# AkiRusProd/numpy-nn-model

Hardware: AMD Instinct MI355X
Metric: samples/sec training step (higher is better)
Workload: dtype f32; 1 GPU; C4: GPT-tiny d512 L6 H8 d_ff2048 vocab15000 training step, batch 64 x seq 256 per GPU, Adam(1.5e-4), dropout 0; global_batch=64, seq_len=256, parallelism=dp1, launch=hipGraph replay, scaling=weak: 64 sequences per GPU

## Files before the change

include/neunet_hip.h:

```cpp
#ifndef NEUNET_HIP_H
#define NEUNET_HIP_H

#include <stdint.h>

#ifdef __cplusplus
extern "C" {
#endif

typedef void* nnhipStream_t;

#define NNHIP_OK 0
#define NNHIP_EINVAL (-1)
#define NNHIP_EALIGN (-2)
#define NNHIP_ENOMEM (-3)
#define NNHIP_EDEVICE (-5)

int nnhipVersion(void);
const char* nnhipGetLastErrorString(void);
int nnhipCleanup(void);
int nnhipDeviceError(void);
int nnhipClearDeviceError(void);
int nnhipRaiseDeviceErrorForTest(int32_t code, nnhipStream_t stream);
int nnhipWorkspaceReserve(int64_t bytes);
int nnhipWorkspaceLock(int locked);

int nnhipSetGemmMode(int mode);
int nnhipGetGemmMode(void);
int nnhipSetGemmLockstep(int enable);
int nnhipGetGemmLockstep(void);
int64_t nnhipGemmLaunchCount(int family);

int nnhipLinearModuleForward(const float* X, const float* W, const float* b, float* O,
                             int64_t rows, int64_t in_features, int64_t out_features,
                             nnhipStream_t stream);
int nnhipLinearModuleBackward(const float* X, const float* W, const float* dO, float* dX,
                              float* dW, float* db, int64_t rows, int64_t in_features,
                              int64_t out_features, nnhipStream_t stream);
int nnhipLinearModuleForwardEx(const float* X, const float* W, const float* b, const float* addend, float* O,
                               int64_t rows, int64_t in_features, int64_t out_features, nnhipStream_t stream);
int nnhipLinearModuleBackwardEx(const float* X, const float* W, const float* dO, const float* dX_addend, float* dX,
                                float* dW, float* db, int64_t rows, int64_t in_features, int64_t out_features,
                                nnhipStream_t stream);

#define NNHIP_LINEAR_GEMV_MAX_ROWS 8
int nnhipLinearGemvForward(const float* X, const float* W, const float* b, const float* addend, float* O, int64_t rows,
                           int64_t in_features, int64_t out_features, nnhipStream_t stream);
int nnhipSetLinearGemv(int enable);
int nnhipGetLinearGemv(void);

int nnhipWeightGradDefer(int32_t enable, nnhipStream_t stream);
int nnhipWeightGradFlush(nnhipStream_t stream);
int nnhipWeightGradFlushGemms(nnhipStream_t stream);
// ... 387 lines not shown
```

numpy-nn-model_amd/csrc/common.h:

```cpp
#pragma once
#include <hip/hip_runtime.h>
#include <stdint.h>
#include <stdio.h>

#include "../../include/neunet_hip.h"

namespace nnhip {

constexpr int kWave = 64;

void set_last_error(const char* fmt, ...);
int hip_status(hipError_t e, const char* what);

#define NNHIP_CHECK_ARG(cond, code, ...)      \
    do {                                       \
        if (!(cond)) {                         \
            nnhip::set_last_error(__VA_ARGS__); \
            return (code);                     \
        }                                      \
    } while (0)

#define NNHIP_LAUNCH_CHECK(name)                          \
    do {                                                  \
        hipError_t _e = hipGetLastError();                \
// ... 2 lines not shown

inline bool aligned16(const void* p) { return (reinterpret_cast<uintptr_t>(p) & 15u) == 0; }
inline bool aligned8(const void* p) { return (reinterpret_cast<uintptr_t>(p) & 7u) == 0; }
inline bool aligned4(const void* p) { return (reinterpret_cast<uintptr_t>(p) & 3u) == 0; }
inline int64_t ceil_div(int64_t a, int64_t b) { return (a + b - 1) / b; }

void* workspace(size_t bytes);
void* workspace_arena(int which, size_t bytes);
bool workspace_locked();
bool wgrad_defer_on();
int conv_reduce_flush(void* stream);
void conv_reduce_cleanup();
int colsum_flush(void* stream);
void colsum_cleanup();
struct WgradJob {
    const float* A; const float* B; float* C; float* asum;
    int64_t M, N, K;
};

const float* zero_block();
constexpr int kSyncWords = 1024;
enum SyncSlot { SYNC_CE = 0, SYNC_MLP = 24 };
unsigned* sync_words();
enum DeviceErrorCode { NNHIP_DEVERR_NONE = 0, NNHIP_DEVERR_MLP_BARRIER = 1, NNHIP_DEVERR_LSTM_SHAPE = 2, NNHIP_DEVERR_KVCACHE_FULL = 3, NNHIP_DEVERR_RECURRENT_SHAPE = 4 };
unsigned* device_error_word();
int device_error_status(const char* who);
int serialize_shared_state(hipStream_t st);
void shared_state_done(hipStream_t st);
struct SharedStateUse {
    hipStream_t st;
    explicit SharedStateUse(hipStream_t s) : st(s) {}
    ~SharedStateUse() { shared_state_done(st); }
    SharedStateUse(const SharedStateUse&) = delete;
    SharedStateUse& operator=(const SharedStateUse&) = delete;
};

template <int CTRL>
__device__ __forceinline__ float dpp_f32(float v) {
    return __builtin_bit_cast(float, __builtin_amdgcn_update_dpp(0, __builtin_bit_cast(int, v), CTRL, 0xF, 0xF, false));
}
template <int CTRL>
__device__ __forceinline__ int dpp_i32(int v) { return __builtin_amdgcn_update_dpp(0, v, CTRL, 0xF, 0xF, false); }
constexpr int kDppXor1 = 0xB1, kDppXor2 = 0x4E, kDppHalfMirror = 0x141, kDppMirror = 0x140;
__device__ __forceinline__ float readlane_f32(float v, int lane) {
    return __builtin_bit_cast(float, __builtin_amdgcn_readlane(__builtin_bit_cast(int, v), lane));
}
// ... 97 lines not shown
```

numpy-nn-model_amd/csrc/gemm.hip:

```cpp
#include <stdlib.h>

#include <type_traits>

#include "gemm_common.h"

namespace nnhip {

__device__ int g_gemm_progress[8192];


template <int BK, bool AKC, bool BKC, bool VEC, bool SUM>
__device__ __forceinline__ void gemm_k_loop(f32x16 (&acc)[2][2], float4 (&ra)[BK / 8], float4 (&rb)[BK / 8], float4& cs,
                                            float* __restrict__ smem, const float* __restrict__ A,
                                            const float* __restrict__ B, const GemmParams& p, int nk, int64_t kbeg,
                                            int64_t kend, int64_t m0, int64_t n0, int tid, int wm, int wn, int l31,
                                            int lh, const float* __restrict__ Z) {
    using TA = Tile<BK, AKC>;
    using TB = Tile<BK, BKC>;
    constexpr int STAGE = TA::SIZE + TB::SIZE;
    constexpr int NLD = 2 * (BK / 8);
    constexpr int NMF = 16 * (BK / 8);
    int cur = 0;
    for (int kt = 0; kt < nk; ++kt) {
        const bool more = kt + 1 < nk;
// ... 107 lines not shown
                                         int l31, int lh) {
    using TA = Tile<BK, AKC>;
    using TB = Tile<BK, BKC>;
    const float* As = smem + cur * (TA::SIZE + TB::SIZE);
    const float* Bs = As + TA::SIZE;
#pragma unroll 1
    for (int g = g0; g < BK / 8; ++g) {
        float a[2][4], b[2][4];
#pragma unroll
        for (int i = 0; i < 2; ++i) {
            frag<BK, AKC>(a[i], As, wm * 64 + i * 32 + l31, g, lh);
            frag<BK, BKC>(b[i], Bs, wn * 64 + i * 32 + l31, g, lh);
        }
#pragma unroll
        for (int j = 0; j < 4; ++j)
#pragma unroll
            for (int i = 0; i < 2; ++i)
#pragma unroll
                for (int n = 0; n < 2; ++n)
                    acc[i][n] = __builtin_amdgcn_mfma_f32_32x32x2f32(a[i][j], b[n][j], acc[i][n], 0, 0, 0);
    }
}

template <int BK, bool AKC, bool BKC, bool VEC, bool CS = false>
__device__ __forceinline__ void gemm_f32_block(const GemmParams& p, const int L, const int by, float* __restrict__ smem) {
    static_assert(!CS || !AKC, "row sums of A are only implemented for an outer-major A");
    using TA = Tile<BK, AKC>;

    const int tid = threadIdx.x;
    const int lane = tid & 63, wave = tid >> 6;
    const int wm = wave >> 1, wn = wave & 1;
    const int l31 = lane & 31, lh = lane >> 5;
#ifdef GEMM_PROF
    long long ts_[5];
    ts_[0] = clock64();
#define GP_STAMP(i) ts_[i] = clock64()
#else
#define GP_STAMP(i) do {} while (0)
#endif
    const int tiles = p.tiles_m * p.tiles_n;
    const int split = L / tiles;
    const int t = L - split * tiles;
    constexpr int GM = 8;
    const int in_group = GM * p.tiles_n;
    const int grp = t / in_group;
    const int first_m = grp * GM;
    const int gsz = min(p.tiles_m - first_m, GM);
// ... 95 lines not shown
            gemm_k_step<BK, AKC, BKC, CS>(acc, ra2, rb2, ra, rb, cs, csf, smem, cur, rsa, rsb, ka_of(kt + 2), kb_of(kt + 2), offa, offb,
                                          tid, wm, wn, l31, lh);
            cur ^= 1;
        }
        if (plock) __builtin_amdgcn_s_setprio(0);
        if (has_tail) {
            tail_mma<BK, AKC, BKC>(acc, smem, cur, (BK - rem) >> 3, wm, wn, l31, lh);
            __syncthreads();
        }
        GP_STAMP(2);
    } else {
        const int nk = (int)((kend - kbeg + BK - 1) / BK);
        const float* __restrict__ Z = p.zeros;
        g2r<BK, AKC, VEC>(ra, A, p.lda, p.M, kend, m0, kbeg, tid, nk > 0, Z);
        g2r<BK, BKC, VEC>(rb, B, p.ldb, p.N, kend, n0, kbeg, tid, nk > 0, Z);
        r2s<BK, AKC>(ra, smem, tid);
        r2s<BK, BKC>(rb, smem + TA::SIZE, tid);
        __syncthreads();
        gemm_k_loop<BK, AKC, BKC, VEC, CS>(acc, ra, rb, cs, smem, A, B, p, nk, kbeg, kend, m0, n0, tid, wm, wn, l31, lh, Z);
    }

#ifdef GEMM_PROF
    long long ets_[5] = {0, 0, 0, 0, 0};
    gemm_epilogue<CS>(acc, p, smem, cs, tid, wave, lane, wm, wn, l31, lh, m0, n0, tn, split, c_off, ets_);
#else
    gemm_epilogue<CS>(acc, p, smem, cs, tid, wave, lane, wm, wn, l31, lh, m0, n0, tn, split, c_off);
#endif
#ifdef GEMM_PROF
    if constexpr (VEC) {
        GP_STAMP(3);
        __builtin_amdgcn_s_waitcnt(0);
        GP_STAMP(4);
        if (p.prof && lane == 0) {
            long long* o = p.prof + ((int64_t)blockIdx.x * 4 + wave) * 12;
            o[0] = ts_[0]; o[1] = ts_[1]; o[2] = ts_[2]; o[3] = ts_[3]; o[4] = ts_[4];
            for (int q_ = 0; q_ < 5; ++q_) o[5 + q_] = ets_[q_];
            o[10] = __builtin_amdgcn_s_getreg((31 << 11) | 4);
            o[11] = ((long long)__builtin_amdgcn_s_getreg((31 << 11) | 20) << 32) | (unsigned)(tm * 65536 + tn);
        }
    }
#endif
}

template <int BK, bool AKC, bool BKC, bool VEC, bool CS = false>
__global__ __launch_bounds__(NT, (BK <= 16) ? 3 : 2) void gemm_f32_kernel(const GemmParams p) {
    extern __shared__ __attribute__((aligned(16))) float smem[];
    gemm_f32_block<BK, AKC, BKC, VEC, CS>(p, xcd_order((int)blockIdx.x, (int)gridDim.x), (int)blockIdx.y, smem);
}

template <int BK>
__global__ __launch_bounds__(NT, 2) void gemm_f32_group_kernel(const GemmGroup g) {
    extern __shared__ __attribute__((aligned(16))) float smem[];
    const int b = (int)blockIdx.x;
    const int L = g.by_job ? b : xcd_order(b, (int)gridDim.x);
    int i = 0;
#pragma unroll
    for (int j = 1; j < GEMM_GROUP_MAX; ++j)
        if (j < g.n && L >= g.start[j]) i = j;
    const int local = L - g.start[i];
    gemm_f32_block<BK, false, false, true, true>(g.p[i], g.by_job ? xcd_order(local, g.start[i + 1] - g.start[i]) : local, 0, smem);
}

struct ReduceArgs {
    const float* slab; float* C; float* preact; const float* bias;
    int64_t M, N, ldc;
    int splitk, act; float beta, alpha;
    const float* asum_slab; float* asum; const float* addend; int asum_blocks, vec;
    const float* dswish; int dact;
};
__device__ __forceinline__ void splitk_reduce_body(const ReduceArgs& r, const int blk, const int nblk) {
    const float* __restrict__ slab = r.slab; float* __restrict__ C = r.C; float* __restrict__ preact = r.preact;
    const float* __restrict__ bias = r.bias; const float* __restrict__ asum_slab = r.asum_slab; float* __restrict__ asum = r.asum;
    const float* __restrict__ addend = r.addend; const float* __restrict__ dswish = r.dswish;
    const int64_t M = r.M, N = r.N, ldc = r.ldc;
    const int splitk = r.splitk, act = r.act, vec = r.vec, dact = r.dact;
    const float beta = r.beta, alpha = r.alpha;
    const int64_t total = M * N;
    const int main_blocks = nblk - r.asum_blocks;
    if (blk >= main_blocks) {
        const int64_t i = (int64_t)(blk - main_blocks) * blockDim.x + threadIdx.x;
        if (i < M) {
            float s = 0.f;
            for (int k = 0; k < splitk; ++k) s += asum_slab[(int64_t)k * M + i];
// ... 80 lines not shown
        hipError_t e = hipFuncSetAttribute(reinterpret_cast<const void*>(kern),
                                           hipFuncAttributeMaxDynamicSharedMemorySize, (int)lds);
        if (e != hipSuccess) return hip_status(e, "hipFuncSetAttribute(gemm)");
        attr_set = true;
    }
    dim3 grid((unsigned)(p.tiles_m * p.tiles_n * p.splitk), (unsigned)batch);
    hipLaunchKernelGGL(kern, grid, dim3(NT), lds, st, p);
    NNHIP_LAUNCH_CHECK("gemm_f32_kernel");
    return 0;
}

int gemm_f32_ex(const float* A, const float* B, float* C, const float* bias, float* preact, int64_t M,
                int64_t N, int64_t K, int64_t lda, int64_t ldb, int64_t ldc, bool a_kmajor, bool b_kmajor,
                int64_t batch1, int64_t sA, int64_t sB, int64_t sC, int64_t batch2, int64_t sA2,
                int64_t sB2, int64_t sC2, float alpha, int act, float beta, hipStream_t st, float* asum = nullptr,
                const float* addend = nullptr, const float* dswish = nullptr, int dact = 1);

int gemm_bf3_launch(const GemmParams& p, bool a_kmajor, bool b_kmajor, bool vec, bool cs, int64_t batch, hipStream_t st);
int gemm_bf3_group_launch(const GemmGroup& g, int blocks, hipStream_t st);
long long linear_gemv_launches();
static int gemm_f32_uneven_split(const float* A, const float* B, float* C, float* asum, int64_t M, int64_t N, int64_t K, int64_t lda,
                                 int64_t ldb, int64_t ldc, int64_t K1, hipStream_t st);
static long long g_gemm_launches[4] = {0, 0, 0, 0};
static int g_gemm_lockstep = []() { const char* e = getenv("NNHIP_GEMM_LOCKSTEP"); return e && atoi(e) == 1 ? 1 : 0; }();
static int g_gemm_mode = -1;
static int gemm_mode() {
    if (g_gemm_mode < 0) {
        const char* e = getenv("NNHIP_GEMM_MODE");
        g_gemm_mode = (e && (atoi(e) == 1 || e[0] == 'b')) ? 1 : 0;
    }
    return g_gemm_mode;
}

bool gemm_pst_wanted(int64_t M, int64_t N, int64_t K, int64_t lda, int64_t ldb, int64_t ldc, const float* A, const float* B,
                     const float* C, const float* bias, bool b_kmajor, int act, const float* preact, const float* dswish, int dact);
int gemm_pst(const float* A, const float* B, float* C, const float* bias, float* preact, int64_t M, int64_t N, int64_t K,
             int64_t lda, int64_t ldb, int64_t ldc, bool b_kmajor, float alpha, int act, float beta, const float* dswish, int dact,
             hipStream_t st);
int gemm_small_linear_backward(const float* X, const float* W, const float* dO, float* dX, float* dW, float* db, int64_t rows,
                               int64_t in, int64_t out, const float* addend, const float* dact_arg, int dact, float beta,
                               hipStream_t st);
bool gemm_small_wanted(int64_t M, int64_t N, int64_t K, int64_t batch, int64_t lda, int64_t ldb, bool a_kmajor, bool b_kmajor);
int gemm_small(const float* A, const float* B, float* C, const float* bias, float* preact, int64_t M, int64_t N, int64_t K,
               int64_t lda, int64_t ldb, int64_t ldc, bool a_kmajor, bool b_kmajor, float alpha, int act, float beta,
               float* asum, const float* addend, const float* dact_arg, int dact, hipStream_t st);

#ifdef GEMM_PROF
static long long* g_gemm_prof = nullptr;
// ... 196 lines not shown
    constexpr int BK = 32;
    const size_t floats = 2 * (size_t)(M * N + (asum ? M : 0));
    float* slab = static_cast<float*>(workspace(floats * sizeof(float)));
    if (!slab) { set_last_error("split-K workspace allocation failed"); return NNHIP_ENOMEM; }
    const float* zeros = zero_block();
    if (!zeros) { set_last_error("zero block allocation failed"); return NNHIP_ENOMEM; }
    float* asum_slab = asum ? slab + 2 * (size_t)(M * N) : nullptr;
    GemmGroup g{};
    g.n = 2;
    g.by_job = 1;
    const int tiles_m = (int)ceil_div(M, BM), tiles_n = (int)ceil_div(N, BN), tiles = tiles_m * tiles_n;
    for (int i = 0; i < 2; ++i) {
        GemmParams& p = g.p[i];
        const int64_t k0 = i ? K1 : 0, kn = i ? K - K1 : K1;
        p.A = A + k0 * lda; p.B = B + k0 * ldb; p.C = C; p.M = M; p.N = N; p.K = kn; p.lda = lda; p.ldb = ldb; p.ldc = ldc;
        p.batch2 = 1; p.alpha = 1.f; p.beta = 1.f; p.tiles_m = tiles_m; p.tiles_n = tiles_n;
        p.k_per_split = ceil_div(kn, BK) * BK;
        p.splitk = 2;
        p.slab = slab + (size_t)i * M * N; p.zeros = zeros; p.cvec = 1; p.asum = asum;
        p.asum_slab = asum ? asum_slab + (size_t)i * M : nullptr;
        g.start[i] = i * tiles;
    }
    for (int i = 2; i <= GEMM_GROUP_MAX; ++i) g.start[i] = 2 * tiles;
    if (int rc = launch_group(g, 2 * tiles, st)) return rc;
    const int rvec = (ldc & 3) == 0 && aligned16(C);
    const int64_t work = rvec ? M * N / 4 : M * N;
    const int blocks = (int)(ceil_div(work, 256) < 2048 ? ceil_div(work, 256) : 2048);
    const int asum_blocks = asum ? (int)ceil_div(M, 256) : 0;
    const ReduceArgs r{slab, C, nullptr, nullptr, M, N, ldc, 2, ACT_NONE, 1.f, 1.f, asum_slab, asum, nullptr, asum_blocks, rvec, nullptr, 0};
    hipLaunchKernelGGL(splitk_reduce_kernel, dim3(blocks + asum_blocks), dim3(256), 0, st, r);
    NNHIP_LAUNCH_CHECK("splitk_reduce_kernel");
    return 0;
}

static int64_t wgrad_chunk(int64_t K) {
    static const int64_t forced = []() { const char* e = getenv("NNHIP_WGRAD_CHUNK"); return (int64_t)(e ? atoi(e) : 0); }();
    if (forced > 0) return ceil_div(forced, (int64_t)32) * 32;
    const int64_t c = ceil_div(ceil_div(K, (int64_t)4), (int64_t)32) * 32;
    return c < 1024 ? 1024 : c;
}
bool gemm_f32_wgrad_group_ok(const WgradJob& j) {
    static const int on = []() { const char* e = getenv("NNHIP_WGRAD_GROUP_KERNEL"); return e ? atoi(e) : 1; }();
    if (!on) return false;
    if (j.M <= 0 || j.N <= 0 || j.K < 4096 || (j.K & 7)) return false;
    if ((j.M & 3) || (j.N & 3) || !aligned16(j.A) || !aligned16(j.B) || !aligned16(j.C)) return false;
    if (j.K * j.M + 128 >= ((int64_t)1 << 30) || j.K * j.N + 128 >= ((int64_t)1 << 30)) return false;
    const int64_t tiles = ceil_div(j.M, BM) * ceil_div(j.N, BN);
    return tiles <= 256;
}

int gemm_f32_wgrad_group(const WgradJob* jobs, int n, hipStream_t st) {
    if (n <= 0) return 0;
    if (n > GEMM_GROUP_MAX) {
        for (int i = 0; i < n; i += GEMM_GROUP_MAX)
            if (int rc = gemm_f32_wgrad_group(jobs + i, n - i < GEMM_GROUP_MAX ? n - i : GEMM_GROUP_MAX, st)) return rc;
        return 0;
    }
    GemmGroup g{};
    ReduceGroup rg{};
    size_t floats = 0;
    for (int i = 0; i < n; ++i) {
        const WgradJob& j = jobs[i];
        const int64_t kps = wgrad_chunk(j.K);
        floats += (size_t)ceil_div(j.K, kps) * (size_t)(j.M * j.N + (j.asum ? j.M : 0));
    }
    float* slab = static_cast<float*>(workspace_arena(1, floats * sizeof(float)));
    if (!slab) { set_last_error("grouped dW workspace allocation failed"); return NNHIP_ENOMEM; }
    const float* zeros = zero_block();
    if (!zeros) { set_last_error("zero block allocation failed"); return NNHIP_ENOMEM; }
    g.n = rg.n = n;
    int blocks = 0, rblocks = 0;
    for (int i = 0; i < n; ++i) {
        const WgradJob& j = jobs[i];
        GemmParams& p = g.p[i];
        p = GemmParams{};
        p.A = j.A; p.B = j.B; p.C = j.C; p.M = j.M; p.N = j.N; p.K = j.K; p.lda = j.M; p.ldb = j.N; p.ldc = j.N;
        p.batch2 = 1; p.alpha = 1.f; p.beta = 1.f;
        p.tiles_m = (int)ceil_div(j.M, BM); p.tiles_n = (int)ceil_div(j.N, BN);
        p.k_per_split = wgrad_chunk(j.K);
        p.splitk = (int)ceil_div(j.K, p.k_per_split);
        p.slab = slab; p.zeros = zeros; p.cvec = 1; p.asum = j.asum;
        slab += (size_t)p.splitk * j.M * j.N;
        if (j.asum) { p.asum_slab = slab; slab += (size_t)p.splitk * j.M; }
        g.start[i] = blocks;
        blocks += p.tiles_m * p.tiles_n * p.splitk;
        const int64_t work = j.M * j.N / 4;
        const int main_blocks = (int)(ceil_div(work, 256) < 2048 ? ceil_div(work, 256) : 2048);
        const int asum_blocks = j.asum ? (int)ceil_div(j.M, 256) : 0;
        rg.r[i] = ReduceArgs{p.slab, j.C, nullptr, nullptr, j.M, j.N, j.N, p.splitk, ACT_NONE, 1.f, 1.f, p.asum_slab, j.asum, nullptr,
                             asum_blocks, 1, nullptr, 0};
        rg.start[i] = rblocks;
        rblocks += main_blocks + asum_blocks;
    }
    for (int i = n; i <= GEMM_GROUP_MAX; ++i) { g.start[i] = blocks; rg.start[i] = rblocks; }
    g_gemm_launches[gemm_mode() == 1 ? 3 : 0] += n;
    if (int rc = launch_group(g, blocks, st)) return rc;
    hipLaunchKernelGGL(splitk_reduce_group_kernel, dim3((unsigned)rblocks), dim3(256), 0, st, rg);
    NNHIP_LAUNCH_CHECK("splitk_reduce_group_kernel");
    return 0;
}

}

extern "C" int nnhipSetGemmMode(int mode) {
    NNHIP_CHECK_ARG(mode == 0 || mode == 1, NNHIP_EINVAL, "nnhipSetGemmMode: 0 = exact fp32 MFMA, 1 = split-bf16 (bf16x3)");
    nnhip::g_gemm_mode = mode;
    return 0;
}
extern "C" int nnhipGetGemmMode(void) { return nnhip::gemm_mode(); }
extern "C" int nnhipSetGemmLockstep(int enable) {
    NNHIP_CHECK_ARG(enable == 0 || enable == 1, NNHIP_EINVAL, "nnhipSetGemmLockstep: 0 = off (default), 1 = the two blocks of a CU keep step");
    nnhip::g_gemm_lockstep = enable;
    return 0;
}
extern "C" int nnhipGetGemmLockstep(void) { return nnhip::g_gemm_lockstep; }
extern "C" int64_t nnhipGemmLaunchCount(int family) {
    if (family == 4) return (int64_t)nnhip::linear_gemv_launches();
    return family >= 0 && family < 4 ? (int64_t)nnhip::g_gemm_launches[family] : -1;
}

extern "C" int nnhipGemmF32Ex(const float* A, const float* B, float* C, const float* bias, int64_t M,
                              int64_t N, int64_t K, int64_t lda, int64_t ldb, int64_t ldc, int a_kmajor,
                              int b_kmajor, int64_t batch1, int64_t sA1, int64_t sB1, int64_t sC1,
                              int64_t batch2, int64_t sA2, int64_t sB2, int64_t sC2, float alpha,
                              nnhipStream_t stream) {
    NNHIP_CHECK_ARG(A && B && C, NNHIP_EINVAL, "nnhipGemmF32Ex: null operand");
    NNHIP_CHECK_ARG(M >= 0 && N >= 0 && K >= 0 && batch1 >= 0 && batch2 >= 1, NNHIP_EINVAL, "nnhipGemmF32Ex: bad size");
    NNHIP_CHECK_ARG(batch1 * batch2 <= 65535, NNHIP_EINVAL, "nnhipGemmF32Ex: batch1*batch2 must be <= 65535");
    NNHIP_CHECK_ARG(nnhip::aligned4(A) && nnhip::aligned4(B) && nnhip::aligned4(C), NNHIP_EALIGN,
                    "nnhipGemmF32Ex: pointers must be 4-byte aligned");
    return nnhip::gemm_f32_ex(A, B, C, bias, nullptr, M, N, K, lda, ldb, ldc, a_kmajor != 0, b_kmajor != 0,
                              batch1, sA1, sB1, sC1, batch2, sA2, sB2, sC2, alpha, nnhip::ACT_NONE, 1.f,
                              static_cast<hipStream_t>(stream));
}

extern "C" int nnhipGemmF32(const float* A, const float* B, float* C, const float* bias, int64_t M,
                            int64_t N, int64_t K, int64_t lda, int64_t ldb, int64_t ldc,
                            int a_kmajor, int b_kmajor, int64_t batch, int64_t strideA,
// ... 11 lines not shown
```

numpy-nn-model_amd/csrc/gemm_common.h:

```cpp
#pragma once
#include "common.h"

namespace nnhip {

typedef float f32x16 __attribute__((ext_vector_type(16)));

enum { ACT_NONE = 0, ACT_SWISH = 1, ACT_RELU = 2, ACT_SIGMOID = 3,
       ACT_SWISH_D = 4 };

struct GemmParams {
    const float* A;
    const float* B;
    float* C;
    const float* bias;
    float* preact;
    int64_t M, N, K, lda, ldb, ldc, sA, sB, sC;
    int64_t sA2, sB2, sC2;
    int batch2;
    float alpha;
    int tiles_m, tiles_n, splitk;
    int lockstep = 0;
#ifdef GEMM_PROF
    long long* prof;
#endif
    int64_t k_per_split;
    float* slab;
    const float* zeros;
    int cvec;
    int act;
    float beta;
    const float* dswish;
    int dact;
    const float* addend;
    float* asum;
    float* asum_slab;
};

constexpr int BM = 128, BN = 128, NT = 256;

template <int BK, bool KC, bool VEC>
__device__ __forceinline__ void g2r(float4 (&r)[BK / 8], const float* __restrict__ P, int64_t ld,
                                    int64_t R, int64_t Kend, int64_t r0, int64_t k0, int tid, bool live,
                                    const float* __restrict__ Z) {
#pragma unroll
    for (int p = 0; p < BK / 8; ++p) {
        const int idx = tid + NT * p;
        int64_t gr, gk;
        const float* src;
        if constexpr (KC) {
            const int rr = idx / (BK / 4), k4 = (idx % (BK / 4)) * 4;
            gr = r0 + rr; gk = k0 + k4;
            src = P + gr * ld + gk;
        } else {
            const int kk = idx / 32, r4 = (idx % 32) * 4;
            gk = k0 + kk; gr = r0 + r4;
            src = P + gk * ld + gr;
        }
        if constexpr (VEC) {
// ... 54 lines not shown
#pragma unroll
    for (int p = 0; p < BK / 8; ++p) {
        const int idx = tid + NT * p;
        if constexpr (KC) {
            const int rr = idx / (BK / 4), k4 = (idx % (BK / 4)) * 4;
            const int64_t rc = min((int64_t)rr, R - 1 - r0);
            off[p] = (unsigned)((rc * ld + k4) * 4);
        } else {
            const int kk = idx / 32, r4 = (idx % 32) * 4;
            const int64_t rc = min((int64_t)r4, R - 4 - r0);
            off[p] = (unsigned)(((int64_t)kk * ld + rc) * 4);
        }
    }
}
template <int BK>
__device__ __forceinline__ void g2r_fast(float4 (&r)[BK / 8], __amdgpu_buffer_rsrc_t rs, unsigned koff, const unsigned (&off)[BK / 8]) {
#pragma unroll
    for (int p = 0; p < BK / 8; ++p) {
        const u32x4_ t = __builtin_amdgcn_raw_buffer_load_b128(rs, off[p], koff, 0);
        r[p].x = __uint_as_float(t.x); r[p].y = __uint_as_float(t.y); r[p].z = __uint_as_float(t.z); r[p].w = __uint_as_float(t.w);
    }
}

template <bool CS>
__device__ __forceinline__ void gemm_epilogue(f32x16 (&acc)[2][2], const GemmParams& p, float* __restrict__ smem, float4 cs,
                                              int tid, int wave, int lane, int wm, int wn, int l31, int lh, int64_t m0,
                                              int64_t n0, int tn, int split, int64_t c_off, long long* ets = nullptr) {
    const bool to_slab = p.splitk > 1;
    if constexpr (CS) {
        if (p.asum && tn == 0) {
            *reinterpret_cast<float4*>(&smem[(tid >> 5) * 128 + (tid & 31) * 4]) = cs;
            __syncthreads();
            if (tid < 128) {
                float t = 0.f;
#pragma unroll
                for (int r = 0; r < 8; ++r) t += smem[r * 128 + tid];
                if (m0 + tid < p.M) (to_slab ? p.asum_slab + (int64_t)split * p.M : p.asum)[m0 + tid] = t;
            }
            __syncthreads();
        }
    }
    float* __restrict__ C = to_slab ? p.slab + (int64_t)split * p.M * p.N : p.C + c_off;
    const int64_t ldc = to_slab ? p.N : p.ldc;
    if (p.cvec) {
        constexpr int ELD = 68;
        float* E = smem + wave * (32 * ELD);
        const int er = lane >> 4, ec = (lane & 15) * 4;
        const int64_t col = n0 + wn * 64 + ec;
        const bool col_ok = col < p.N;
        float4 bv = make_float4(0.f, 0.f, 0.f, 0.f);
        if (!to_slab && p.bias && col_ok) bv = *reinterpret_cast<const float4*>(p.bias + col);
        const float* __restrict__ extra = to_slab ? nullptr : (p.addend ? p.addend : p.dswish);
        const bool is_add = p.addend != nullptr;
        float4 ex[8];
        auto fetch_extra = [&](int i, int it) {
            const int64_t row = m0 + wm * 64 + i * 32 + it * 4 + er;
            ex[it] = make_float4(0.f, 0.f, 0.f, 0.f);
            if (row < p.M && col_ok) ex[it] = *reinterpret_cast<const float4*>(extra + c_off + row * ldc + col);
        };
        if (extra) {
#pragma unroll
            for (int it = 0; it < 8; ++it) fetch_extra(0, it);
        }
#ifdef GEMM_PROF
        if (ets) ets[0] = clock64();
#endif
#pragma unroll
        for (int i = 0; i < 2; ++i) {
#pragma unroll
            for (int n = 0; n < 2; ++n)
#pragma unroll
                for (int e = 0; e < 16; ++e)
                    E[((e & 3) + 8 * (e >> 2) + 4 * lh) * ELD + n * 32 + l31] = acc[i][n][e];
            __builtin_amdgcn_s_waitcnt(0xc07f);
            __builtin_amdgcn_wave_barrier();
#ifdef GEMM_PROF
// ... 18 lines not shown
                                v.z = x.z > 0.f ? v.z : 0.f; v.w = x.w > 0.f ? v.w : 0.f;
                            } else if (p.dact == 3) {
                                v.x *= x.x; v.y *= x.y; v.z *= x.z; v.w *= x.w;
                            } else {
                                v.x *= swish_grad_(x.x, p.beta); v.y *= swish_grad_(x.y, p.beta);
                                v.z *= swish_grad_(x.z, p.beta); v.w *= swish_grad_(x.w, p.beta);
                            }
                        }
                        if (p.act == ACT_SWISH) {
                            if (p.preact) *reinterpret_cast<float4*>(p.preact + c_off + row * ldc + col) = v;
                            v.x *= sigmoid_fast_(p.beta * v.x); v.y *= sigmoid_fast_(p.beta * v.y);
                            v.z *= sigmoid_fast_(p.beta * v.z); v.w *= sigmoid_fast_(p.beta * v.w);
                        } else if (p.act == ACT_SWISH_D) {
                            float4 d;
                            swish_fwd_d_(v.x, p.beta, v.x, d.x); swish_fwd_d_(v.y, p.beta, v.y, d.y);
                            swish_fwd_d_(v.z, p.beta, v.z, d.z); swish_fwd_d_(v.w, p.beta, v.w, d.w);
                            if (p.preact) *reinterpret_cast<float4*>(p.preact + c_off + row * ldc + col) = d;
                        } else if (p.act == ACT_RELU) {
                            v.x = fmaxf(v.x, 0.f); v.y = fmaxf(v.y, 0.f); v.z = fmaxf(v.z, 0.f); v.w = fmaxf(v.w, 0.f);
                        } else if (p.act == ACT_SIGMOID) {
                            v.x = sigmoid_fast_(v.x); v.y = sigmoid_fast_(v.y); v.z = sigmoid_fast_(v.z); v.w = sigmoid_fast_(v.w);
                        }
                    }
                    *reinterpret_cast<float4*>(C + row * ldc + col) = v;
                }
            }
            __builtin_amdgcn_s_waitcnt(0xc07f);
            __builtin_amdgcn_wave_barrier();
#ifdef GEMM_PROF
            if (ets) ets[2 + 2 * i] = clock64();
#endif
        }
        return;
    }
#pragma unroll
    for (int n = 0; n < 2; ++n) {
        const int64_t col = n0 + wn * 64 + n * 32 + l31;
        if (col >= p.N) continue;
        const float bv = (!to_slab && p.bias) ? p.bias[col] : 0.f;
#pragma unroll
        for (int i = 0; i < 2; ++i) {
            const int64_t rbase = m0 + wm * 64 + i * 32 + 4 * lh;
#pragma unroll
            for (int e = 0; e < 16; ++e) {
                const int64_t row = rbase + (e & 3) + 8 * (e >> 2);
                if (row >= p.M) continue;
                float v = to_slab ? acc[i][n][e] : p.alpha * acc[i][n][e] + bv;
// ... 2 lines not shown
                    if (p.dswish) {
                        const float x = p.dswish[c_off + row * ldc + col];
                        v = p.dact == 2 ? (x > 0.f ? v : 0.f) : p.dact == 3 ? v * x : v * swish_grad_(x, p.beta);
                    }
                    if (p.act == ACT_SWISH) {
                        if (p.preact) p.preact[c_off + row * ldc + col] = v;
                        v = v * sigmoid_fast_(p.beta * v);
                    } else if (p.act == ACT_SWISH_D) {
                        float d;
                        swish_fwd_d_(v, p.beta, v, d);
                        if (p.preact) p.preact[c_off + row * ldc + col] = d;
                    } else if (p.act == ACT_RELU) {
                        v = fmaxf(v, 0.f);
                    } else if (p.act == ACT_SIGMOID) {
                        v = sigmoid_fast_(v);
                    }
                }
                C[row * ldc + col] = v;
            }
        }
    }
}

__device__ __forceinline__ int xcd_order(int b, int nwg) {
    const int xcd = b & 7, q = nwg >> 3, r = nwg & 7;
    return (xcd < r ? xcd * (q + 1) : r * (q + 1) + (xcd - r) * q) + (b >> 3);
}


constexpr int GEMM_GROUP_MAX = 8;
struct GemmGroup {
    GemmParams p[GEMM_GROUP_MAX];
    int start[GEMM_GROUP_MAX + 1];
    int n;
    int by_job;
};

}
```

numpy-nn-model_amd/csrc/runtime.hip:

```cpp
#include <stdarg.h>
#include <string.h>

#include <mutex>

#include "common.h"

namespace nnhip {

static thread_local char g_err[512] = "";

void set_last_error(const char* fmt, ...) {
    va_list ap;
    va_start(ap, fmt);
    vsnprintf(g_err, sizeof(g_err), fmt, ap);
    va_end(ap);
}

int hip_status(hipError_t e, const char* what) {
    if (e == hipSuccess) return 0;
    set_last_error("%s: %s (%d)", what, hipGetErrorString(e), (int)e);
    return (int)e;
}

static std::mutex g_ws_mu;
// ... 114 lines not shown
        default: return "unknown device error code";
    }
}
int device_error_status(const char* who) {
    if (!g_deverr_host) return 0;
    const unsigned code = *const_cast<volatile unsigned*>(g_deverr_host);
    if (code == NNHIP_DEVERR_NONE) return 0;
    set_last_error("%s: device error %u raised by an earlier kernel -- %s (nnhipClearDeviceError() resets it)", who, code, device_error_text(code));
    return NNHIP_EDEVICE;
}

unsigned* sync_words() {
    static unsigned* w = nullptr;
    static std::once_flag once;
    std::call_once(once, []() {
        unsigned* p = nullptr;
        if (hipMalloc(reinterpret_cast<void**>(&p), kSyncWords * sizeof(unsigned)) == hipSuccess &&
            hipMemset(p, 0, kSyncWords * sizeof(unsigned)) == hipSuccess)
            w = p;
    });
    return w;
}

}

extern "C" int nnhipVersion(void) { return 221; }

extern "C" int nnhipDeviceError(void) { return nnhip::device_error_status("nnhipDeviceError"); }

extern "C" int nnhipClearDeviceError(void) {
    if (nnhip::g_deverr_host) *const_cast<volatile unsigned*>(nnhip::g_deverr_host) = 0u;
    return 0;
}

__global__ void raise_device_error_kernel(unsigned* err, unsigned code) {
    if (err) __hip_atomic_store(err, code, __ATOMIC_RELAXED, __HIP_MEMORY_SCOPE_SYSTEM);
}
extern "C" int nnhipRaiseDeviceErrorForTest(int32_t code, nnhipStream_t stream) {
    unsigned* w = nnhip::device_error_word();
    if (!w) { nnhip::set_last_error("nnhipRaiseDeviceErrorForTest: no device error word (pinned allocation failed)"); return NNHIP_ENOMEM; }
    hipLaunchKernelGGL(raise_device_error_kernel, dim3(1), dim3(64), 0, (hipStream_t)stream, w, (unsigned)code);
    NNHIP_LAUNCH_CHECK("raise_device_error_kernel");
    return 0;
}

extern "C" int nnhipWorkspaceReserve(int64_t bytes) {
    if (bytes < 0) { nnhip::set_last_error("nnhipWorkspaceReserve: negative size"); return NNHIP_EINVAL; }
    if (bytes > 0 && !nnhip::workspace((size_t)bytes)) return NNHIP_ENOMEM;
    return 0;
// ... 29 lines not shown
```

numpy-nn-model_amd/neunet_hip/_lib.py:

```python
from __future__ import annotations

import ctypes
import os
from ctypes import POINTER, c_char, c_double, c_float, c_int32, c_int64, c_void_p

_HERE = os.path.dirname(os.path.abspath(__file__))
LIB_ENV = "NEUNET_HIP_LIB"
DEFAULT_LIB = os.path.join(_HERE, "lib", "libneunet_hip.so")


class NeunetHipError(RuntimeError):
    """Raised for any non-zero status from libneunet_hip.so."""


class Conv2dDesc(ctypes.Structure):
    _fields_ = [(n, c_int64) for n in ("B", "Cin", "H", "W", "Cout", "kh", "kw", "sh", "sw", "dh", "dw",
                                       "pu", "pd", "pl", "pr")]


class ConvTranspose2dDesc(ctypes.Structure):
    _fields_ = [(n, c_int64) for n in ("B", "Cin", "H", "W", "Cout", "kh", "kw", "sh", "sw", "dh", "dw",
                                       "pu", "pd", "pl", "pr", "oph", "opw")]


# ... 22 lines not shown
    _fields_ = [("dwx", c_void_p * 3), ("dwh", c_void_p * 3), ("db", c_void_p * 3)]


class RNNWeights(ctypes.Structure):
    _fields_ = [("wx", c_void_p), ("wh", c_void_p), ("b", c_void_p)]


class RNNGrads(ctypes.Structure):
    _fields_ = [("dwx", c_void_p), ("dwh", c_void_p), ("db", c_void_p)]


P = c_void_p
_SIGNATURES = {
    "nnhipVersion": (ctypes.c_int, []),
    "nnhipGetLastErrorString": (ctypes.c_char_p, []),
    "nnhipCleanup": (ctypes.c_int, []),
    "nnhipDeviceError": (ctypes.c_int, []),
    "nnhipClearDeviceError": (ctypes.c_int, []),
    "nnhipRaiseDeviceErrorForTest": (ctypes.c_int, [ctypes.c_int32, ctypes.c_void_p]),
    "nnhipSetGemmMode": (ctypes.c_int, [ctypes.c_int]),
    "nnhipGetGemmMode": (ctypes.c_int, []),
    "nnhipSetGemmLockstep": (ctypes.c_int, [ctypes.c_int]),
    "nnhipGetGemmLockstep": (ctypes.c_int, []),
    "nnhipGemmLaunchCount": (c_int64, [ctypes.c_int]),
    "nnhipWorkspaceReserve": (ctypes.c_int, [c_int64]),
    "nnhipWorkspaceLock": (ctypes.c_int, [ctypes.c_int]),
    "nnhipLinearModuleForward": (ctypes.c_int, [P, P, P, P, c_int64, c_int64, c_int64, c_void_p]),
    "nnhipLinearModuleBackward": (ctypes.c_int, [P, P, P, P, P, P, c_int64, c_int64, c_int64, c_void_p]),
    "nnhipWeightGradDefer": (ctypes.c_int, [ctypes.c_int32, c_void_p]),
    "nnhipWeightGradFlush": (ctypes.c_int, [c_void_p]),
    "nnhipWeightGradFlushGemms": (ctypes.c_int, [c_void_p]),
    "nnhipWeightGradPending": (ctypes.c_int, []),
    "nnhipLinearInputGradSwish": (ctypes.c_int, [P, P, P, P, c_int64, c_int64, c_int64, c_float, c_void_p]),
    "nnhipLinearInputGradScaled": (ctypes.c_int, [P, P, P, P, c_int64, c_int64, c_int64, c_void_p]),
    "nnhipLinearInputGradReLU": (ctypes.c_int, [P, P, P, P, c_int64, c_int64, c_int64, c_void_p]),
    "nnhipLinearReLULinearBackward": (ctypes.c_int, [P, P, P, P, P, P, P, P, c_int64, c_int64, c_int64, c_int64, c_void_p]),
    "nnhipLinearReLULinearBackwardAdam": (ctypes.c_int, [P, P, P, P, P, P, P, P, c_int64, c_int64, c_int64, c_int64, c_void_p,
                                                          ctypes.POINTER(c_void_p), ctypes.c_double, ctypes.c_double, ctypes.c_double,
                                                          ctypes.c_double, ctypes.c_double, ctypes.c_int32, ctypes.c_int32, c_float, c_void_p]),
    "nnhipLinearReLULinearBackwardFits": (ctypes.c_int, [c_int64, c_int64, c_int64, c_int64, ctypes.c_int32]),
    "nnhipLinearModuleBackwardAct": (ctypes.c_int, [P, P, P, P, c_int32, c_float, P, P, P, c_int64, c_int64, c_int64, c_void_p]),
    "nnhipLinearActivationForward": (ctypes.c_int, [P, P, P, P, c_int64, c_int64, c_int64, c_int32, c_float, c_void_p]),
    "nnhipLinearModuleForwardEx": (ctypes.c_int, [P, P, P, P, P, c_int64, c_int64, c_int64, c_void_p]),
    "nnhipLinearModuleBackwardEx": (ctypes.c_int, [P, P, P, P, P, P, P, c_int64, c_int64, c_int64, c_void_p]),
    "nnhipLinearGemvForward": (ctypes.c_int, [P, P, P, P, P, c_int64, c_int64, c_int64, c_void_p]),
    "nnhipSetLinearGemv": (ctypes.c_int, [ctypes.c_int]),
# ... 111 lines not shown
    "nnhipMSELossSigmoidForwardBackward": (ctypes.c_int, [P, P, P, P, c_int64, c_void_p]),
    "nnhipBatchNorm1dForward": (ctypes.c_int, [P, P, P, P, P, P, P, P, c_int64, c_int64, c_float, c_float, ctypes.c_int, c_void_p]),
    "nnhipBatchNorm1dBackward": (ctypes.c_int, [P, P, P, P, P, P, P, P, c_int64, c_int64, c_void_p]),
    "nnhipTanhForward": (ctypes.c_int, [P, P, c_int64, c_void_p]),
    "nnhipTanhBackward": (ctypes.c_int, [P, P, P, c_int64, c_void_p]),
    "nnhipBCELossForwardBackward": (ctypes.c_int, [P, P, P, c_float, P, P, c_int64, c_char, ctypes.c_int, c_void_p]),
    "nnhipGaussianReparamForward": (ctypes.c_int, [P, P, P, P, P, c_int64, c_void_p]),
    "nnhipGaussianReparamBackward": (ctypes.c_int, [P, P, P, P, P, c_int64, c_void_p]),
    "nnhipGaussianKLDForwardBackward": (ctypes.c_int, [P, P, P, P, P, c_int64, c_void_p]),
    "nnhipVQNearest": (ctypes.c_int, [P, P, P, P, c_int64, c_int64, c_int64, c_void_p]),
    "nnhipVQLossForwardBackward": (ctypes.c_int, [P, P, c_float, P, P, P, c_int64, c_void_p]),
    "nnhipScale": (ctypes.c_int, [P, c_float, c_int64, c_void_p]),
    "nnhipScaleRows": (ctypes.c_int, [P, P, P, c_int64, c_int64, c_int64, c_void_p]),
    "nnhipAdd": (ctypes.c_int, [P, P, P, c_int64, c_void_p]),
    "nnhipCommUniqueId": (ctypes.c_int, [ctypes.c_char_p]),
    "nnhipCommInitRank": (ctypes.c_int, [POINTER(c_void_p), ctypes.c_char_p, ctypes.c_int, ctypes.c_int]),
    "nnhipCommDestroy": (ctypes.c_int, [c_void_p]),
    "nnhipCommRank": (ctypes.c_int, [c_void_p, POINTER(ctypes.c_int), POINTER(ctypes.c_int)]),
    "nnhipCommLibrary": (ctypes.c_int, [ctypes.c_char_p, c_int64, POINTER(ctypes.c_int)]),
    "nnhipAllReduceSumF32": (ctypes.c_int, [c_void_p, P, c_int64, c_void_p]),
    "nnhipAllReduceAvgF32": (ctypes.c_int, [c_void_p, P, c_int64, c_void_p]),
    "nnhipBroadcastF32": (ctypes.c_int, [c_void_p, P, c_int64, ctypes.c_int, c_void_p]),
}
_NO_STATUS = {"nnhipVersion", "nnhipLinearReLULinearBackwardFits", "nnhipBatchNorm2dLinearSigmoidMSEFits", "nnhipConv2dLeakyMaxPoolStatsBlocks", "nnhipGetLastErrorString", "nnhipCreateFusedOptimizer", "nnhipGetGemmMode", "nnhipGetGemmLockstep", "nnhipConv2dWeightGradPooledOk", "nnhipConv2dLeakyMaxPoolForwardOk", "nnhipGemmLaunchCount",
              "nnhipWeightGradPending", "nnhipGetLinearGemv", "nnhipSetConvTransposeRoute", "nnhipGetConvTransposeRoute",
              "nnhipConvTranspose2dPlan"}

_dll = None
_funcs: dict = {}


def lib_path() -> str:
    return os.environ.get(LIB_ENV, DEFAULT_LIB)


def load_library():
    global _dll
    if _dll is None:
        path = lib_path()
        if not os.path.exists(path):
            raise NeunetHipError(
                f"libneunet_hip.so not found at {path!r}; build it with "
                f"`python numpy-nn-model_amd/build.py` (or set ${LIB_ENV}). There is no CPU fallback.")
        _dll = ctypes.CDLL(path, mode=ctypes.RTLD_GLOBAL)
    return _dll


# ... 136 lines not shown
```

Measured before the change: 3029 samples/s.

## Reduce split-K weight-gradient partials in-kernel via per-tile tickets

Replaces the separate split-K reduce launch after grouped weight-gradient GEMMs with an in-kernel scheme. Each block writes its partial tile, increments an atomic ticket, and the last block to arrive for that tile sums all the slabs and writes C and the row sums. This removes one kernel launch and its serialization gap per grouped dW call. In exchange it adds atomic and fence overhead in the epilogue, leaves the reduction on whichever block arrives last (which can lengthen the tail), and relies on the ticket words being reset correctly.

```diff
diff --git a/include/neunet_hip.h b/include/neunet_hip.h
--- a/include/neunet_hip.h
+++ b/include/neunet_hip.h
@@ -28,6 +28,10 @@
 int nnhipGetGemmMode(void);
 int nnhipSetGemmLockstep(int enable);
 int nnhipGetGemmLockstep(void);
+int nnhipSetWgradInKernelReduce(int enable);
+int nnhipGetWgradInKernelReduce(void);
+int nnhipGemmTicketsNonzero(int32_t which);
+int64_t nnhipWgradInKernelReduceCount(void);
 int64_t nnhipGemmLaunchCount(int family);
 
 int nnhipLinearModuleForward(const float* X, const float* W, const float* b, float* O,
diff --git a/numpy-nn-model_amd/csrc/common.h b/numpy-nn-model_amd/csrc/common.h
--- a/numpy-nn-model_amd/csrc/common.h
+++ b/numpy-nn-model_amd/csrc/common.h
@@ -48,6 +48,8 @@
 constexpr int kSyncWords = 1024;
 enum SyncSlot { SYNC_CE = 0, SYNC_MLP = 24 };
 unsigned* sync_words();
+constexpr int kGemmTicketWords = 4096;
+unsigned* gemm_tickets(int which);
 enum DeviceErrorCode { NNHIP_DEVERR_NONE = 0, NNHIP_DEVERR_MLP_BARRIER = 1, NNHIP_DEVERR_LSTM_SHAPE = 2, NNHIP_DEVERR_KVCACHE_FULL = 3, NNHIP_DEVERR_RECURRENT_SHAPE = 4 };
 unsigned* device_error_word();
 int device_error_status(const char* who);
diff --git a/numpy-nn-model_amd/csrc/gemm.hip b/numpy-nn-model_amd/csrc/gemm.hip
--- a/numpy-nn-model_amd/csrc/gemm.hip
+++ b/numpy-nn-model_amd/csrc/gemm.hip
@@ -153,7 +153,7 @@
     }
 }
 
-template <int BK, bool AKC, bool BKC, bool VEC, bool CS = false>
+template <int BK, bool AKC, bool BKC, bool VEC, bool CS = false, bool TK = false>
 __device__ __forceinline__ void gemm_f32_block(const GemmParams& p, const int L, const int by, float* __restrict__ smem) {
     static_assert(!CS || !AKC, "row sums of A are only implemented for an outer-major A");
     using TA = Tile<BK, AKC>;
@@ -295,10 +295,14 @@
 
 #ifdef GEMM_PROF
     long long ets_[5] = {0, 0, 0, 0, 0};
-    gemm_epilogue<CS>(acc, p, smem, cs, tid, wave, lane, wm, wn, l31, lh, m0, n0, tn, split, c_off, ets_);
+    gemm_epilogue<CS, TK>(acc, p, smem, cs, tid, wave, lane, wm, wn, l31, lh, m0, n0, tn, split, c_off, ets_);
 #else
-    gemm_epilogue<CS>(acc, p, smem, cs, tid, wave, lane, wm, wn, l31, lh, m0, n0, tn, split, c_off);
+    gemm_epilogue<CS, TK>(acc, p, smem, cs, tid, wave, lane, wm, wn, l31, lh, m0, n0, tn, split, c_off);
 #endif
+    if constexpr (TK) {
+        if (p.tickets && tile_ticket_arrive(p.tickets + (tm * p.tiles_n + tn), (unsigned)p.red_need, smem, tid))
+            splitk_tile_sum(p, tid, m0, n0, tn);
+    }
 #ifdef GEMM_PROF
     if constexpr (VEC) {
         GP_STAMP(3);
@@ -331,7 +335,7 @@
     for (int j = 1; j < GEMM_GROUP_MAX; ++j)
         if (j < g.n && L >= g.start[j]) i = j;
     const int local = L - g.start[i];
-    gemm_f32_block<BK, false, false, true, true>(g.p[i], g.by_job ? xcd_order(local, g.start[i + 1] - g.start[i]) : local, 0, smem);
+    gemm_f32_block<BK, false, false, true, true, true>(g.p[i], g.by_job ? xcd_order(local, g.start[i + 1] - g.start[i]) : local, 0, smem);
 }
 
 struct ReduceArgs {
@@ -458,8 +462,10 @@
 static int gemm_f32_uneven_split(const float* A, const float* B, float* C, float* asum, int64_t M, int64_t N, int64_t K, int64_t lda,
                                  int64_t ldb, int64_t ldc, int64_t K1, hipStream_t st);
 static long long g_gemm_launches[4] = {0, 0, 0, 0};
+static long long g_ticket_jobs = 0;
 static int g_gemm_lockstep = []() { const char* e = getenv("NNHIP_GEMM_LOCKSTEP"); return e && atoi(e) == 1 ? 1 : 0; }();
 static int g_gemm_mode = -1;
+static int g_inkernel_reduce = []() { const char* e = getenv("NNHIP_WGRAD_INKERNEL_REDUCE"); return e ? (atoi(e) != 0 ? 1 : 0) : 1; }();
 static int gemm_mode() {
     if (g_gemm_mode < 0) {
         const char* e = getenv("NNHIP_GEMM_MODE");
@@ -702,8 +708,16 @@
         g.start[i] = i * tiles;
     }
     for (int i = 2; i <= GEMM_GROUP_MAX; ++i) g.start[i] = 2 * tiles;
+    const int rvec = (ldc & 3) == 0 && aligned16(C);
+    unsigned* tk = g_inkernel_reduce && gemm_mode() == 0 && rvec && tiles <= kGemmTicketWords ? gemm_tickets(0) : nullptr;
+    if (tk) {
+        for (int i = 0; i < 2; ++i) {
+            g.p[i].tickets = tk; g.p[i].red_need = 2; g.p[i].red_slab = slab; g.p[i].red_asum_slab = asum_slab;
+        }
+        ++g_ticket_jobs;
+        return launch_group(g, 2 * tiles, st);
+    }
     if (int rc = launch_group(g, 2 * tiles, st)) return rc;
-    const int rvec = (ldc & 3) == 0 && aligned16(C);
     const int64_t work = rvec ? M * N / 4 : M * N;
     const int blocks = (int)(ceil_div(work, 256) < 2048 ? ceil_div(work, 256) : 2048);
     const int asum_blocks = asum ? (int)ceil_div(M, 256) : 0;
@@ -749,7 +763,9 @@
     const float* zeros = zero_block();
     if (!zeros) { set_last_error("zero block allocation failed"); return NNHIP_ENOMEM; }
     g.n = rg.n = n;
-    int blocks = 0, rblocks = 0;
+    int blocks = 0, rblocks = 0, tiles = 0;
+    for (int i = 0; i < n; ++i) tiles += (int)(ceil_div(jobs[i].M, BM) * ceil_div(jobs[i].N, BN));
+    unsigned* tk = g_inkernel_reduce && gemm_mode() == 0 && tiles <= kGemmTicketWords ? gemm_tickets(1) : nullptr;
     for (int i = 0; i < n; ++i) {
         const WgradJob& j = jobs[i];
         GemmParams& p = g.p[i];
@@ -762,6 +778,11 @@
         p.slab = slab; p.zeros = zeros; p.cvec = 1; p.asum = j.asum;
         slab += (size_t)p.splitk * j.M * j.N;
         if (j.asum) { p.asum_slab = slab; slab += (size_t)p.splitk * j.M; }
+        if (tk && p.splitk > 1) {
+            p.tickets = tk; p.red_need = p.splitk; p.red_slab = p.slab; p.red_asum_slab = p.asum_slab;
+            tk += p.tiles_m * p.tiles_n;
+            ++g_ticket_jobs;
+        }
         g.start[i] = blocks;
         blocks += p.tiles_m * p.tiles_n * p.splitk;
         const int64_t work = j.M * j.N / 4;
@@ -775,6 +796,7 @@
     for (int i = n; i <= GEMM_GROUP_MAX; ++i) { g.start[i] = blocks; rg.start[i] = rblocks; }
     g_gemm_launches[gemm_mode() == 1 ? 3 : 0] += n;
     if (int rc = launch_group(g, blocks, st)) return rc;
+    if (tk) return 0;
     hipLaunchKernelGGL(splitk_reduce_group_kernel, dim3((unsigned)rblocks), dim3(256), 0, st, rg);
     NNHIP_LAUNCH_CHECK("splitk_reduce_group_kernel");
     return 0;
@@ -794,6 +816,13 @@
     return 0;
 }
 extern "C" int nnhipGetGemmLockstep(void) { return nnhip::g_gemm_lockstep; }
+extern "C" int nnhipSetWgradInKernelReduce(int enable) {
+    NNHIP_CHECK_ARG(enable == 0 || enable == 1, NNHIP_EINVAL, "nnhipSetWgradInKernelReduce: 0 = a reduce launch behind the grid, 1 = summed by the last block of a tile (default)");
+    nnhip::g_inkernel_reduce = enable;
+    return 0;
+}
+extern "C" int nnhipGetWgradInKernelReduce(void) { return nnhip::g_inkernel_reduce; }
+extern "C" int64_t nnhipWgradInKernelReduceCount(void) { return (int64_t)nnhip::g_ticket_jobs; }
 extern "C" int64_t nnhipGemmLaunchCount(int family) {
     if (family == 4) return (int64_t)nnhip::linear_gemv_launches();
     return family >= 0 && family < 4 ? (int64_t)nnhip::g_gemm_launches[family] : -1;
diff --git a/numpy-nn-model_amd/csrc/gemm_common.h b/numpy-nn-model_amd/csrc/gemm_common.h
--- a/numpy-nn-model_amd/csrc/gemm_common.h
+++ b/numpy-nn-model_amd/csrc/gemm_common.h
@@ -34,6 +34,10 @@
     const float* addend;
     float* asum;
     float* asum_slab;
+    unsigned* tickets = nullptr;
+    const float* red_slab = nullptr;
+    const float* red_asum_slab = nullptr;
+    int red_need = 0;
 };
 
 constexpr int BM = 128, BN = 128, NT = 256;
@@ -134,7 +138,7 @@
     }
 }
 
-template <bool CS>
+template <bool CS, bool WT = false>
 __device__ __forceinline__ void gemm_epilogue(f32x16 (&acc)[2][2], const GemmParams& p, float* __restrict__ smem, float4 cs,
                                               int tid, int wave, int lane, int wm, int wn, int l31, int lh, int64_t m0,
                                               int64_t n0, int tn, int split, int64_t c_off, long long* ets = nullptr) {
@@ -147,7 +151,11 @@
                 float t = 0.f;
 #pragma unroll
                 for (int r = 0; r < 8; ++r) t += smem[r * 128 + tid];
-                if (m0 + tid < p.M) (to_slab ? p.asum_slab + (int64_t)split * p.M : p.asum)[m0 + tid] = t;
+                if (m0 + tid < p.M) {
+                    float* dst = (to_slab ? p.asum_slab + (int64_t)split * p.M : p.asum) + (m0 + tid);
+                    if (WT && p.tickets) __hip_atomic_store(dst, t, __ATOMIC_RELAXED, __HIP_MEMORY_SCOPE_AGENT);
+                    else *dst = t;
+                }
             }
             __syncthreads();
         }
@@ -164,6 +172,7 @@
         if (!to_slab && p.bias && col_ok) bv = *reinterpret_cast<const float4*>(p.bias + col);
         const float* __restrict__ extra = to_slab ? nullptr : (p.addend ? p.addend : p.dswish);
         const bool is_add = p.addend != nullptr;
+        [[maybe_unused]] const __amdgpu_buffer_rsrc_t wt_rsrc = operand_rsrc(C);
         float4 ex[8];
         auto fetch_extra = [&](int i, int it) {
             const int64_t row = m0 + wm * 64 + i * 32 + it * 4 + er;
@@ -228,7 +237,13 @@
                             v.x = sigmoid_fast_(v.x); v.y = sigmoid_fast_(v.y); v.z = sigmoid_fast_(v.z); v.w = sigmoid_fast_(v.w);
                         }
                     }
-                    *reinterpret_cast<float4*>(C + row * ldc + col) = v;
+                    if (WT && p.tickets) {
+                        u32x4_ u;
+                        u.x = __float_as_uint(v.x); u.y = __float_as_uint(v.y); u.z = __float_as_uint(v.z); u.w = __float_as_uint(v.w);
+                        __builtin_amdgcn_raw_buffer_store_b128(u, wt_rsrc, (unsigned)((row * ldc + col) * 4), 0, 16);
+                    } else {
+                        *reinterpret_cast<float4*>(C + row * ldc + col) = v;
+                    }
                 }
             }
             __builtin_amdgcn_s_waitcnt(0xc07f);
@@ -277,6 +292,90 @@
     }
 }
 
+__device__ __forceinline__ bool tile_ticket_arrive(unsigned* word, unsigned need, float* smem, int tid) {
+    asm volatile("s_waitcnt vmcnt(0)" ::: "memory");
+    __syncthreads();
+    if (tid == 0) {
+        const unsigned t = __hip_atomic_fetch_add(word, 1u, __ATOMIC_RELAXED, __HIP_MEMORY_SCOPE_AGENT);
+        const bool last = t == need - 1u;
+        if (last) {
+            __builtin_amdgcn_fence(__ATOMIC_ACQUIRE, "agent");
+            asm volatile("s_waitcnt vmcnt(0)" ::: "memory");
+            __hip_atomic_store(word, 0u, __ATOMIC_RELAXED, __HIP_MEMORY_SCOPE_AGENT);
+        }
+        reinterpret_cast<unsigned*>(smem)[0] = last ? 1u : 0u;
+    }
+    __syncthreads();
+    return reinterpret_cast<const unsigned*>(smem)[0] != 0u;
+}
+
+__device__ __forceinline__ void splitk_tile_sum(const GemmParams& p, int tid, int64_t m0, int64_t n0, int tn) {
+    const int need = p.red_need;
+    const int64_t MN = p.M * p.N;
+    const float* __restrict__ S = p.red_slab;
+    const int64_t col = n0 + (tid & 31) * 4;
+    const int r0 = tid >> 5;
+    if (col < p.N) {
+#pragma unroll 1
+        for (int b = 0; b < 4; ++b) {
+            float4 s[4];
+            int64_t off[4];
+            bool ok[4];
+#pragma unroll
+            for (int q = 0; q < 4; ++q) {
+                const int64_t row = m0 + r0 + 8 * (b * 4 + q);
+                ok[q] = row < p.M;
+                off[q] = (ok[q] ? row : m0) * p.N + col;
+                s[q] = make_float4(0.f, 0.f, 0.f, 0.f);
+            }
+            int k = 0;
+            for (; k + 4 <= need; k += 4) {
+                float4 v[4][4];
+#pragma unroll
+                for (int j = 0; j < 4; ++j)
+#pragma unroll
+                    for (int q = 0; q < 4; ++q) v[j][q] = *reinterpret_cast<const float4*>(S + (int64_t)(k + j) * MN + off[q]);
+#pragma unroll
+                for (int q = 0; q < 4; ++q) {
+                    s[q].x = (((s[q].x + v[0][q].x) + v[1][q].x) + v[2][q].x) + v[3][q].x;
+                    s[q].y = (((s[q].y + v[0][q].y) + v[1][q].y) + v[2][q].y) + v[3][q].y;
+                    s[q].z = (((s[q].z + v[0][q].z) + v[1][q].z) + v[2][q].z) + v[3][q].z;
+                    s[q].w = (((s[q].w + v[0][q].w) + v[1][q].w) + v[2][q].w) + v[3][q].w;
+                }
+            }
+            for (; k + 2 <= need; k += 2) {
+                float4 v[2][4];
+#pragma unroll
+                for (int j = 0; j < 2; ++j)
+#pragma unroll
+                    for (int q = 0; q < 4; ++q) v[j][q] = *reinterpret_cast<const float4*>(S + (int64_t)(k + j) * MN + off[q]);
+#pragma unroll
+                for (int q = 0; q < 4; ++q) {
+                    s[q].x = (s[q].x + v[0][q].x) + v[1][q].x; s[q].y = (s[q].y + v[0][q].y) + v[1][q].y;
+                    s[q].z = (s[q].z + v[0][q].z) + v[1][q].z; s[q].w = (s[q].w + v[0][q].w) + v[1][q].w;
+                }
+            }
+            for (; k < need; ++k) {
+#pragma unroll
+                for (int q = 0; q < 4; ++q) {
+                    const float4 v = *reinterpret_cast<const float4*>(S + (int64_t)k * MN + off[q]);
+                    s[q].x += v.x; s[q].y += v.y; s[q].z += v.z; s[q].w += v.w;
+                }
+            }
+#pragma unroll
+            for (int q = 0; q < 4; ++q) {
+                const int64_t row = m0 + r0 + 8 * (b * 4 + q);
+                if (ok[q]) *reinterpret_cast<float4*>(p.C + row * p.ldc + col) = s[q];
+            }
+        }
+    }
+    if (p.asum && tn == 0 && tid < 128 && m0 + tid < p.M) {
+        float s = 0.f;
+        for (int k = 0; k < need; ++k) s += p.red_asum_slab[(int64_t)k * p.M + m0 + tid];
+        p.asum[m0 + tid] = s;
+    }
+}
+
 __device__ __forceinline__ int xcd_order(int b, int nwg) {
     const int xcd = b & 7, q = nwg >> 3, r = nwg & 7;
     return (xcd < r ? xcd * (q + 1) : r * (q + 1) + (xcd - r) * q) + (b >> 3);
diff --git a/numpy-nn-model_amd/csrc/runtime.hip b/numpy-nn-model_amd/csrc/runtime.hip
--- a/numpy-nn-model_amd/csrc/runtime.hip
+++ b/numpy-nn-model_amd/csrc/runtime.hip
@@ -160,9 +160,38 @@
     return w;
 }
 
-}
-
-extern "C" int nnhipVersion(void) { return 221; }
+unsigned* gemm_tickets(int which) {
+    static unsigned* w[2] = {nullptr, nullptr};
+    static std::once_flag once;
+    std::call_once(once, []() {
+        unsigned* p = nullptr;
+        if (hipMalloc(reinterpret_cast<void**>(&p), 2 * kGemmTicketWords * sizeof(unsigned)) == hipSuccess &&
+            hipMemset(p, 0, 2 * kGemmTicketWords * sizeof(unsigned)) == hipSuccess) {
+            w[0] = p;
+            w[1] = p + kGemmTicketWords;
+        }
+    });
+    return w[which];
+}
+
+}
+
+extern "C" int nnhipVersion(void) { return 222; }
+
+extern "C" int nnhipGemmTicketsNonzero(int32_t which) {
+    NNHIP_CHECK_ARG(which == 0 || which == 1, NNHIP_EINVAL, "nnhipGemmTicketsNonzero: which is 0 (general workspace) or 1 (grouped dW launch)");
+    unsigned* w = nnhip::gemm_tickets(which);
+    if (!w) { nnhip::set_last_error("nnhipGemmTicketsNonzero: ticket allocation failed"); return NNHIP_ENOMEM; }
+    static unsigned host[nnhip::kGemmTicketWords];
+    static std::mutex mu;
+    std::lock_guard<std::mutex> lk(mu);
+    hipError_t e = hipDeviceSynchronize();
+    if (e == hipSuccess) e = hipMemcpy(host, w, sizeof(host), hipMemcpyDeviceToHost);
+    if (e != hipSuccess) { const int rc = nnhip::hip_status(e, "nnhipGemmTicketsNonzero"); return rc > 0 ? -rc : rc; }
+    int n = 0;
+    for (int i = 0; i < nnhip::kGemmTicketWords; ++i) n += host[i] != 0u;
+    return n;
+}
 
 extern "C" int nnhipDeviceError(void) { return nnhip::device_error_status("nnhipDeviceError"); }
 
diff --git a/numpy-nn-model_amd/neunet_hip/_lib.py b/numpy-nn-model_amd/neunet_hip/_lib.py
--- a/numpy-nn-model_amd/neunet_hip/_lib.py
+++ b/numpy-nn-model_amd/neunet_hip/_lib.py
@@ -68,6 +68,10 @@
     "nnhipGetGemmMode": (ctypes.c_int, []),
     "nnhipSetGemmLockstep": (ctypes.c_int, [ctypes.c_int]),
     "nnhipGetGemmLockstep": (ctypes.c_int, []),
+    "nnhipSetWgradInKernelReduce": (ctypes.c_int, [ctypes.c_int]),
+    "nnhipGetWgradInKernelReduce": (ctypes.c_int, []),
+    "nnhipGemmTicketsNonzero": (ctypes.c_int, [c_int32]),
+    "nnhipWgradInKernelReduceCount": (c_int64, []),
     "nnhipGemmLaunchCount": (c_int64, [ctypes.c_int]),
     "nnhipWorkspaceReserve": (ctypes.c_int, [c_int64]),
     "nnhipWorkspaceLock": (ctypes.c_int, [ctypes.c_int]),
@@ -225,7 +229,7 @@
     "nnhipAllReduceAvgF32": (ctypes.c_int, [c_void_p, P, c_int64, c_void_p]),
     "nnhipBroadcastF32": (ctypes.c_int, [c_void_p, P, c_int64, ctypes.c_int, c_void_p]),
 }
-_NO_STATUS = {"nnhipVersion", "nnhipLinearReLULinearBackwardFits", "nnhipBatchNorm2dLinearSigmoidMSEFits", "nnhipConv2dLeakyMaxPoolStatsBlocks", "nnhipGetLastErrorString", "nnhipCreateFusedOptimizer", "nnhipGetGemmMode", "nnhipGetGemmLockstep", "nnhipConv2dWeightGradPooledOk", "nnhipConv2dLeakyMaxPoolForwardOk", "nnhipGemmLaunchCount",
+_NO_STATUS = {"nnhipVersion", "nnhipLinearReLULinearBackwardFits", "nnhipBatchNorm2dLinearSigmoidMSEFits", "nnhipConv2dLeakyMaxPoolStatsBlocks", "nnhipGetLastErrorString", "nnhipCreateFusedOptimizer", "nnhipGetGemmMode", "nnhipGetGemmLockstep", "nnhipGetWgradInKernelReduce", "nnhipGemmTicketsNonzero", "nnhipWgradInKernelReduceCount", "nnhipConv2dWeightGradPooledOk", "nnhipConv2dLeakyMaxPoolForwardOk", "nnhipGemmLaunchCount",
               "nnhipWeightGradPending", "nnhipGetLinearGemv", "nnhipSetConvTransposeRoute", "nnhipGetConvTransposeRoute",
               "nnhipConvTranspose2dPlan"}
 
```

Result: no change. 3035 samples/s, median of 6 (+0.2%).
